# aleflabo/MoCoDAD

Hardware: AMD Instinct MI355X
Metric: pose-clips/sec (whole node) @ noise_steps=10, 5 seeds; AUC vs ref (higher is better)
Workload: dtype f32

## Files before the change

### mocodad_amd/csrc/mcd_device.hpp

```cpp

#pragma once
#include <hip/hip_runtime.h>
#include <stdint.h>
#include <string.h>
#include <stdlib.h>
#include <math.h>
#include <string>
#include <vector>
#include <unordered_map>
#include <utility>
#include <type_traits>
#include <atomic>

#include "../../include/mocodad_hip.h"
#include "mcd_chain.hpp"

namespace mcd {

typedef float f32x4 __attribute__((ext_vector_type(4)));
typedef float f32x2 __attribute__((ext_vector_type(2)));
typedef const float __attribute__((address_space(4))) cfloat;
typedef const float __attribute__((address_space(1))) gfloat;
typedef const f32x4 __attribute__((address_space(1))) gf32x4;
__device__ __forceinline__ gfloat* as_global(const float* p) { return (gfloat*)p; }
// ... 218 lines not shown
    static constexpr int UNITS = NB * CB * NQ;
    static constexpr int PER = (UNITS + NWAVES - 1) / NWAVES;
    static constexpr int NR = (KS * T + 15) / 16;
    static constexpr bool SAMEQ = NQ == 3 && UNITS == 12 && NWAVES == 8;
    static_assert(T > 12 || PER == 1 || UNITS % NWAVES == 0 || SAMEQ, "mix units: a partial round of units (see MixCfg::QX)");
    __host__ __device__ static constexpr int unit_of(int wave, int round) {
        if constexpr (SAMEQ) {
            if (wave < 4) return (wave >> 1) + NQ * ((wave & 1) * 2 + round);
            return round == 0 ? 2 + NQ * (wave - 4) : -1;
        } else {
            const int u = wave + round * NWAVES;
            return u < UNITS ? u : -1;
        }
    }
};
template <int CIN, int V, int T, int NB>
struct MixCoef {
    using M = MixCfg<CIN, V, T, NB>;
    float tq[M::QC][M::NR], aop[M::QC][M::MT][M::KS];
    __device__ __forceinline__ void load(const float* tqd, const float* af, int wave, int lane) {
        load_unit(tqd, af, M::unit_of(wave, 0), lane);
    }
    __device__ __forceinline__ void load_at(const float* tqd, const float* af, int lane) {
        static_assert(M::QC == 1, "one output frame per unit");
        gfloat* tqd_g = as_global(tqd);
        gfloat* af_g = as_global(af);
#pragma unroll
        for (int r = 0; r < M::NR; ++r) tq[0][r] = tqd_g[r * 64 + lane];
#pragma unroll
        for (int mt = 0; mt < M::MT; ++mt)
// ... 321 lines not shown

template <int MT, int NT>
struct Tiling {
    static constexpr int MW = MT > NWAVES ? MT / NWAVES : 1;
    static constexpr int NG = MT > NWAVES ? 1 : NWAVES / MT;
    static constexpr int MAXN = (NT + NG - 1) / NG;
};
template <int MT, int KQ>
__device__ __forceinline__ void load_afrags(const float4* __restrict__ wp, int wave, int lane, float4 (&a)[KQ], int mi = 0) {
    const float* wpl = reinterpret_cast<const float*>(wp + (((wave + mi * NWAVES) % MT) * KQ) * 64 + lane);
#pragma unroll
    for (int kq = 0; kq < KQ; ++kq) a[kq] = load_global4(wpl + kq * 256);
}

struct NoPre { static constexpr bool none = true; };
template <int MT, int NT, int KQ1, int KQ2, bool IDRES, bool FORCE = false, bool DUAL = FORCE, bool SLOTK = false, class Epi, class Pre = NoPre>
__device__ __forceinline__ void gemm_tiles(const float4 (&a)[KQ1 + KQ2], const float* __restrict__ b1, int cs1,
                                           const float* __restrict__ b2, int cs2, int wave, int lane, Epi&& epi, int mi = 0,
                                           const float4 cinit = make_float4(0.f, 0.f, 0.f, 0.f), Pre&& pre = Pre{}) {
    constexpr bool HASPRE = !std::is_same_v<std::decay_t<Pre>, NoPre>;
    constexpr int NG = Tiling<MT, NT>::NG;
    constexpr int MAXN = Tiling<MT, NT>::MAXN;
    const int mt = (wave + mi * NWAVES) % MT, ng = MT > NWAVES ? 0 : wave / MT;
    if (NWAVES % MT != 0 && MT <= NWAVES && ng >= NG) return;
    const int j = lane & 15, g = lane >> 4;
    const int c0 = mt * 16 + 4 * g;
    const int col0 = ng * 16 + j;
    const float* const p1b = b1 + __mul24(col0, cs1) + 4 * g;
    const float* const p2b = b2 + __mul24(col0, cs2) + 4 * g;
    constexpr int KQ = KQ1 + KQ2;
    constexpr int DEPTH0 = KQ < 3 ? KQ : 3;
    auto one_tile = [&](auto ii) {
        constexpr int i = decltype(ii)::value;
        const int col = col0 + i * NG * 16;
        f32x4 c = {cinit.x, cinit.y, cinit.z, cinit.w};
        const float* p1 = p1b + i * NG * 16 * cs1;
        const float* p2 = p2b + i * NG * 16 * cs2;
        if (IDRES) {
            const float4 r = *reinterpret_cast<const float4*>(p2 - 4 * g + c0);
            c[0] = r.x; c[1] = r.y; c[2] = r.z; c[3] = r.w;
        }
        auto rd = [&](auto kk) {
            constexpr int kq = decltype(kk)::value;
            return *reinterpret_cast<const float4*>(kq < KQ1 ? p1 + kq * 16 : p2 + (kq - KQ1) * 16);
// ... 161 lines not shown
}

struct NoHook { __device__ __forceinline__ void operator()() const {} };

template <int KQ>
struct LayerAfr {
    float4 a[KQ];
    float4 bcur;
    template <int MT, bool U32 = false>
    __device__ __forceinline__ void load(const float* wb, const LayerW& lw, int wave, int lane) {
        load_afrags<MT, KQ>(reinterpret_cast<const float4*>(wptr<U32>(wb, lw.wp)), wave, lane, a);
        bcur = load_global4(wptr<U32>(wb, lw.bias) + (wave % MT) * 16 + 4 * (lane >> 4));
    }
};

template <int CIN, int COUT, int V, bool RES, bool HASEMB, int T, int NB, bool FORCE = false, int CSX = cs_of(CIN), bool SLOTSEL = false, class H1, class H2>
__device__ __forceinline__ void layer_generic(const float* wb, const LayerW lw, const MixCoef<CIN, V, T, NB>& mc,
                                              const float* __restrict__ in, float* __restrict__ z, float* __restrict__ out,
                                              const float* __restrict__ embl, int wave, int lane, Prof& prof, int prof_id,
                                              H1&& pre_gemm, H2&& pre_barrier,
                                              const LayerAfr<(CIN / 16) * (RES ? 2 : 1)>* pre_afr = nullptr, const StageRow* rows = nullptr) {
    constexpr int MT = ceil16(COUT) / 16;
    constexpr int COLS = NB * T * V;
    constexpr int NT = ceil16(COLS) / 16;
    constexpr int TV = T * V;
    constexpr int CSI = cs_of(CIN), CSO = cs_of(COUT);
    constexpr int KQ1 = CIN / 16, KQ2 = RES ? CIN / 16 : 0;
    float4 afr[KQ1 + KQ2];
    const int trs = 8 + 8 * ((prof_id - 32) / 3);
    prof.trace(trs + 0);
    constexpr bool TSEL = SLOTSEL && HASEMB && NB == 2 && T == 3;
    constexpr bool ROWS = TSEL && MixCfg<CIN, V, T, NB>::QC == 1;
    const float* bias = wptr<TSEL>(wb, lw.bias);
    float4 bcur;
    if (pre_afr != nullptr) {
#pragma unroll
        for (int k = 0; k < KQ1 + KQ2; ++k) afr[k] = pre_afr->a[k];
        bcur = pre_afr->bcur;
    } else {
        load_afrags<MT, KQ1 + KQ2>(reinterpret_cast<const float4*>(wptr<TSEL>(wb, lw.wp)), wave, lane, afr);
        bcur = load_global4(bias + (wave % MT) * 16 + 4 * (lane >> 4));
    }
    mix_stage<CIN, V, T, NB, FORCE, HASEMB, ROWS>(in, CSX, mc, wptr<TSEL>(wb, lw.tq), wptr<TSEL>(wb, lw.am), wave, lane,
                             ZeroInit{},
                             [&](int n, int q, int w, auto c, auto v) {
                                 if constexpr (ROWS) {
                                     const unsigned za = c.ob + 4u * (unsigned)(__mul24(w, CSI) + c.j);
                                     if constexpr (std::is_same_v<decltype(v), f32x4>) lds_store4(za, v[0], v[1], v[2], v[3]);
                                     else *(lds_float*)(uintptr_t)za = v;
                                 } else {
                                 float* zp = (z + (n * (T * V) * CSI + q * (V * CSI) + c.cb16)) + (__mul24(w, CSI) + c.j);
                                 if constexpr (std::is_same_v<decltype(v), f32x4>) lds_store4(lds_addr(zp), v[0], v[1], v[2], v[3]);
                                 else *zp = v;
                                 }
                             }, rows);
    prof.trace(trs + 1);
    pre_gemm();
    bsync();
// ... 56 lines not shown
    auto epi = [&](auto ti, int col, int c0, f32x4 acc, int, int ng, auto... pe) {
        if (COUT % 16 == 0 || c0 < COUT) {
            float4 e = make_float4(0.f, 0.f, 0.f, 0.f);
            if constexpr (sizeof...(pe) > 0) e = (pe, ...);
            else if constexpr (HASEMB) e = emb_of(ti, col, ng);
            f32x2 t0 = f32x2{acc[0], acc[1]}, t1 = f32x2{acc[2], acc[3]};
            if constexpr (!FOLD) { t0 += f32x2{bcur.x, bcur.y}; t1 += f32x2{bcur.z, bcur.w}; }
            const f32x2 m0 = t0 * slope, m1 = t1 * slope;
            const f32x2 r0 = f32x2{__builtin_amdgcn_fmed3f(t0[0], m0[0], pinf), __builtin_amdgcn_fmed3f(t0[1], m0[1], pinf)} + f32x2{e.x, e.y};
            const f32x2 r1 = f32x2{__builtin_amdgcn_fmed3f(t1[0], m1[0], pinf), __builtin_amdgcn_fmed3f(t1[1], m1[1], pinf)} + f32x2{e.z, e.w};
            constexpr unsigned tile_bytes = 4u * decltype(ti)::value * TILE_STEP * CSO;
            lds_store4(oaddr + tile_bytes, r0[0], r0[1], r1[0], r1[1]);
        }
    };
    prof.trace(trs + 3);
    if constexpr (EPRE) gemm_tiles<MT, NT, KQ1, KQ2, !RES, FORCE, FORCE, TSEL>(afr, z, CSI, in, CSX, wave, lane, epi, 0, FOLD ? bcur : make_float4(0.f, 0.f, 0.f, 0.f), emb_of);
    else gemm_tiles<MT, NT, KQ1, KQ2, !RES, FORCE, FORCE, TSEL>(afr, z, CSI, in, CSX, wave, lane, epi, 0, FOLD ? bcur : make_float4(0.f, 0.f, 0.f, 0.f));
#pragma unroll
    for (int mi = 1; mi < Tiling<MT, NT>::MW; ++mi) {
        load_afrags<MT, KQ1 + KQ2>(reinterpret_cast<const float4*>(wptr<TSEL>(wb, lw.wp)), wave, lane, afr, mi);
        bcur = load_global4(bias + ((wave + mi * NWAVES) % MT) * 16 + 4 * (lane >> 4));
        set_bases(mi);
        if constexpr (EHOIST) e_pre = lds_load4(eaddr);
        if constexpr (EPRE) gemm_tiles<MT, NT, KQ1, KQ2, !RES, FORCE, FORCE, TSEL>(afr, z, CSI, in, CSX, wave, lane, epi, mi, FOLD ? bcur : make_float4(0.f, 0.f, 0.f, 0.f), emb_of);
        else gemm_tiles<MT, NT, KQ1, KQ2, !RES, FORCE, FORCE, TSEL>(afr, z, CSI, in, CSX, wave, lane, epi, mi, FOLD ? bcur : make_float4(0.f, 0.f, 0.f, 0.f));
    }
    prof.trace(trs + 4);
    pre_barrier();
#ifdef MCD_PROFILE
    asm volatile("s_waitcnt lgkmcnt(0)" ::: "memory");
#endif
    prof.trace(trs + 5);
    bsync();
    prof.trace(trs + 6);
    prof.mark(prof_id + 1);
}
template <int CIN, int COUT, int V, bool RES, bool HASEMB, int T, int NB>
__device__ __forceinline__ void layer_generic(const float* wb, const LayerW lw, const float* __restrict__ in,
                                              float* __restrict__ z, float* __restrict__ out,
                                              const float* __restrict__ embl, int wave, int lane, Prof& prof, int prof_id) {
    MixCoef<CIN, V, T, NB> mc;
    mc.load(wb + lw.tq, wb + lw.am, wave, lane);
    layer_generic<CIN, COUT, V, RES, HASEMB, T, NB>(wb, lw, mc, in, z, out, embl, wave, lane, prof, prof_id, NoHook{}, NoHook{});
}

template <int L, int T, int NB>
using LMix = MixCoef<layer_desc(L).cin, layer_desc(L).V, T, NB>;
template <int L>
using LAfr = LayerAfr<(layer_desc(L).cin / 16) * (layer_desc(L).res ? 2 : 1)>;
template <int L, bool U32 = false>
__device__ __forceinline__ void load_lafr(LAfr<L>& A, const float* wb, int wave, int lane) {
    A.template load<ceil16(layer_desc(L).cout) / 16, U32>(wb, layer_w(wb, L), wave, lane);
}
template <int L, int T, int NB, bool FORCE = false, int CSX = cs_of(layer_desc(L).cin), class H1, class H2>
__device__ __forceinline__ void layer_std(const float* wb, const LMix<L, T, NB>& mc, const float* in, float* z, float* out,
                                          const float* emb, int wave, int lane, Prof& prof, H1&& pre_gemm, H2&& pre_barrier,
                                          const LAfr<L>* pre_afr = nullptr, const StageRow* rows = nullptr) {
    constexpr LDesc D = layer_desc(L);
    layer_generic<D.cin, D.cout, D.V, D.res != 0, true, T, NB, FORCE, CSX, true>(wb, layer_w(wb, L), mc, in, z, out, emb + emb_off(L), wave, lane,
                                                               prof, 32 + 3 * L, pre_gemm, pre_barrier, pre_afr, rows);
}

struct EmbRow {
    float4 w[4];
    float b;
    template <bool U32 = false>
    __device__ __forceinline__ void load(const float* wb, int o) {
        const float* we = wptr<U32>(wb, tab_i(wb, TAB_WE));
#pragma unroll
        for (int q = 0; q < 4; ++q) w[q] = load_global4(we + o * EDIM + 4 * q);
        b = as_global(wptr<U32>(wb, tab_i(wb, TAB_BE)))[o];
    }
};
template <int NB>
// ... 82 lines not shown
```

### mocodad_amd/csrc/mcd_score_kernel.hpp

```cpp
#pragma once
#include "mcd_device.hpp"
#include "mcd_encode_kernel.hpp"
#include "mcd_stage_table.hpp"

namespace mcd {

template <int T, int NB, int MINW, bool LT = false>
__global__ __launch_bounds__(NTHREADS, MINW) void score_kernel(const ScoreParams P) {
    using PL = Plan<T, NB>;
    constexpr int TV17 = T * 17;
    constexpr int COLS17 = NB * TV17;
    extern __shared__ __attribute__((aligned(16))) float smem[];
    float* const RG = smem;
    float* const XT = smem + PL::O_XT;
    float* const EMB = smem + PL::O_EMB;
    float* const E10 = smem + PL::O_E10;
    float* const SEN = E10 + 32;
    float* const ZN = smem + PL::O_ZN;
    int* const WM = reinterpret_cast<int*>(smem + PL::O_WM);
    float* const BIA = smem + PL::O_BIA;
    int* const UPD = reinterpret_cast<int*>(smem + PL::O_UPD);
    float* const ZO = smem + PL::O_ZO;

    const int tid0 = threadIdx.x;
    int tid = tid0;
    int lane = tid & 63;
    int wave = __builtin_amdgcn_readfirstlane(tid >> 6);
    Prof prof;
    prof.off();
#ifdef MCD_PROFILE
    const unsigned long long wg_t0 = __builtin_amdgcn_s_memrealtime();
#endif
    if (P.phase > 0 && blockIdx.x * 2 >= gridDim.x) {
        const unsigned long long t0 = __builtin_readcyclecounter();
        while (__builtin_readcyclecounter() - t0 < (unsigned long long)P.phase * 1024ull) __builtin_amdgcn_s_sleep(32);
    }
    if (P.phase < -15) {
// ... 3 lines not shown
    }
    const int grp = blockIdx.x / P.split, part = blockIdx.x - grp * P.split;
    const int win0 = grp * NB;
    const int Tx = P.n_corrupt;
    auto window_of = [&](int n) { const int b = win0 + n; return b < P.B ? b : P.B - 1; };
    if (threadIdx.x < NB) {
        const int b = window_of(threadIdx.x);
        WM[threadIdx.x] = P.win_mask ? P.win_mask[b] : (int)P.fixed_mask;
        WM[4 + threadIdx.x] = b;
        if (threadIdx.x == 0) { WM[8] = 0; WM[9] = -1; }
    }
    if (threadIdx.x >= 128 && threadIdx.x < 128 + NB * T) {
        const int i = threadIdx.x - 128, n = i / T, t = i % T;
        const int fixed = P.win_mask ? P.win_mask[window_of(n)] : (int)P.fixed_mask;
        const int k = P.win_mask ? (((fixed >> t) & 1) ? -1 : 0) : P.upd_of[t];
        UPD[i] = k < 0 ? -1 : (n * T + (P.win_mask ? t : P.pos_of[k])) * 17;
    }
    static_assert(NB <= 4 && T <= 16 && NB * T <= 16, "tail index packing: 4 bits (chain, frame) | 2 bits chain | 4 bits frame");
    int* const TT = reinterpret_cast<int*>(ZO + PL::ZO);
    float* const CE = reinterpret_cast<float*>(TT + PL::TT);
    float* const LOSSB = CE + PL::CE;
    float* const EXW = LOSSB + PL::LOSS;
    if constexpr (MINW >= 4) {
        if (threadIdx.x == 0) {
            int sh = P.prio_shift;
            if (sh > 0 && P.tune) {
                const int sig = (int)gridDim.x * 1009 + P.S * 31 + P.ns;
                const int ticks = P.tune[1];
                if (P.tune[0] == sig && ticks > 0) {
                    const unsigned v = (unsigned)(((unsigned long long)(unsigned)ticks * (unsigned)(P.prio_rounds > 0 ? P.prio_rounds : 1)) / 6u) | 1u;
                    sh = 31 - __clz((int)v);
                    if ((v >> (sh > 0 ? sh - 1 : 0)) & 1u) ++sh;
                    sh = sh < 10 ? 10 : (sh > 26 ? 26 : sh);
                }
            }
            UPD[15] = sh;
            UPD[14] = (int)(unsigned)__builtin_amdgcn_s_memrealtime();
        }
    }
    for (int u = threadIdx.x; u < EMB_EXTRA * 17; u += NTHREADS) {
        const int r = u / 17, k = u % 17;
        EXW[r * 20 + k] = k < 16 ? P.wbuf[tab_i(P.wbuf, TAB_WE) + (NTHREADS + r) * EDIM + k] : P.wbuf[tab_i(P.wbuf, TAB_BE) + NTHREADS + r];
    }
    for (int u = threadIdx.x; u < COLS17 * C0; u += NTHREADS) {
        const int col = u / C0, n = col / TV17, t = (col / 17) % T, v = col % 17;
        TT[u] = (n * T + t) | (n << 4) | (t << 6) | (v << 10);
    }
    if (threadIdx.x < 64) BIA[threadIdx.x] = P.wbuf[tab_i(P.wbuf, 6 * F_STRIDE + F_BIAS) + threadIdx.x];
    else if (threadIdx.x < 64 + C0) BIA[threadIdx.x] = P.wbuf[tab_i(P.wbuf, 10 * F_STRIDE + F_BIAS) + threadIdx.x - 64];
    else if (threadIdx.x >= 80 && threadIdx.x < 112) BIA[threadIdx.x] = P.wbuf[tab_i(P.wbuf, 8 * F_STRIDE + F_BIAS) + threadIdx.x - 80];
    const int CTV = C0 * Tx * 17;
    const int K = P.ns > 2 ? P.ns - 1 : 1;

    if (P.cond_inkernel) {
        static_assert(CondFastLds<T, NB>::FLOATS <= PL::R, "cond_fast_body's region does not fit the work region zeroed for it");
        int enc_solo = -1;
        do {
            for (int u = tid; u < PL::R; u += NTHREADS) smem[u] = 0.f;
            bsync();
            cond_fast_body<T, NB, (NB > 1)>(P.wbuf, P.dv, [&](int t) { return P.cond_idx[t]; }, P.seg_len, smem, win0, P.B, CE, nullptr, enc_solo);
// ... 97 lines not shown
            float xv[C0];
#pragma unroll
            for (int c = 0; c < C0; ++c) {
                if (solo >= 0 && n != solo) {
                    xv[c] = 0.f;
                } else if (mode == 1) {
                    xv[c] = x_in ? x_in[((b * C0 + c) * T + t) * 17 + v] : 0.f;
                } else if ((fixed >> t) & 1) {
                    xv[c] = load_coord(dv, b, c, fm_src(P, t), v, seg_len);
                } else {
                    const int e = (c * Tx + fm_tx(P, fixed, t)) * 17 + v;
                    if (noise) xv[c] = noise[((size_t)(s * K + 0) * Bq + b) * CTV + e];
                    else xv[c] = philox_normal(seed, (unsigned)e, 0u, (unsigned)s, (unsigned)(first_window + b));
                }
            }
            XT[u * 4 + 0] = xv[0];
            XT[u * 4 + 1] = xv[1];
        }
    }
    bsync();
    {
        EmbRow er;
        er.load(P.wbuf, tid_s);
        silu_row(i_first, tid_s);
        bsync();
        emb_compute<NB>(er, EXW, SEN, EMB, E10 + (i_first & 1) * 16, tid_s);
        bsync();
    }
    LMix<0, T, NB> mc0;
    mc0.load(P.wbuf + tab_i(P.wbuf, F_TQ), P.wbuf + tab_i(P.wbuf, F_AM), wave, lane);
    constexpr bool WEARLY = T <= 4;
    LAfr<0> A0;
    if constexpr (WEARLY) load_lafr<0>(A0, P.wbuf, wave, lane);
    stage_rows_of(wave);
    srows(r0, srow::L0);
    for (int sidx = i_first; sidx >= i_last; --sidx) {
        const float* srow = P.step_table + sidx * (4 + EDIM);
        const float* wb = P.wbuf;
        asm volatile("" : "+s"(wb));
        tid = tid0;
        asm volatile("" : "+v"(tid));
        lane = tid & 63;
        wave = __builtin_amdgcn_readfirstlane(tid >> 6);
        stage_rows_of(wave);
        if constexpr (MINW >= 4) {
// ... 17 lines not shown
                float z[4] = {0.f, 0.f, 0.f, 0.f};
                const int fixed = WM[n];
                const int solo = NB > 1 ? WM[9] : -1;
                if (!((fixed >> t) & 1) && (solo < 0 || n == solo)) {
                    const int b = WM[4 + n];
                    const int tx = fm_tx(P, fixed, t);
                    const int k = P.ns - sidx;
                    if (P.noise) {
                        const float* zp = P.noise + ((size_t)(s * K + k) * P.B + b) * CTV + tx * 17 + v0;
                        z[0] = zp[0]; z[1] = zp[Tx * 17];
                        if (v0 + 1 < 17) { z[2] = zp[1]; z[3] = zp[Tx * 17 + 1]; }
                    } else {
                        philox_normal4(P.seed, (unsigned)(tx * 9 + (v0 >> 1)), (unsigned)k, (unsigned)s, (unsigned)(P.first_window + b), z);
                    }
                }
                float* zo = ZN + ((n * T + t) * 17 + v0) * C0;
                zo[0] = z[0]; zo[1] = z[1];
                if (v0 + 1 < 17) { zo[2] = z[2]; zo[3] = z[3]; }
            }
        };
        noise_part(tid);
        STAGE(0);
        STAGE(1);
#ifdef MCD_PROFILE
        prof.bidx = 0;
        prof.tr_on = prof.won && prof.tr && s == part && sidx == i_first - 1;
        prof.trace(0);
#endif
        auto mixload = [&](auto& mc, int l) { mc.load(wptr<TSEL>(wb, tab_i(wb, l * F_STRIDE + F_TQ)), wptr<TSEL>(wb, tab_i(wb, l * F_STRIDE + F_AM)), wave, lane); };
        auto rsload = [&](auto& rc, int r) { rc.load(wptr<TSEL>(wb, tab_i(wb, TAB_RSW + r)), wptr<TSEL>(wb, tab_i(wb, TAB_RSB + r)), lane); };
        auto wptrb = [&](unsigned bytes) { return reinterpret_cast<const float*>(reinterpret_cast<const char*>(wb) + bytes); };
        auto mixrow_at = [&](auto& mc, int tq, int am, const StageRow& r) { mc.load_at(wptrb(4u * (unsigned)tq + r.tq_o), wptrb(4u * (unsigned)am + r.af_o), lane); };
        auto mixrows = [&](auto& mc, int l, auto& r, int id) {
            if constexpr (TSEL) { srows(r, id); mixrow_at(mc, tab_i(wb, l * F_STRIDE + F_TQ), tab_i(wb, l * F_STRIDE + F_AM), r[0]); }
            else mixload(mc, l);
        };
        auto mix_early = mixload;
        auto rs_early = rsload;
        NoHook nohook;
        constexpr bool EARLY2 = LOWO || T == 6;
        LMix<1, T, NB> mc1;
        LAfr<1> A1; LAfr<2> A2; LAfr<3> A3; LAfr<4> A4; LAfr<5> A5; LAfr<7> A7; LAfr<9> A9;
        auto wearly = [&](auto& A, auto lc) { if constexpr (WEARLY) load_lafr<decltype(lc)::value, TSEL>(A, wb, wave, lane); };
#define MCD_LC(l) std::integral_constant<int, l>{}
        layer_std<0, T, NB, LOWO, 4>(wb, mc0, XT, RG + PL::L0_z, RG + PL::L0_out, EMB, wave, lane, prof,
                            [&] { mixrows(mc1, 1, r1, srow::L1); }, [&] { wearly(A1, MCD_LC(1)); }, WEARLY ? &A0 : nullptr, r0);
        STAGE(2);
        lt_dump(0, RG + PL::L0_out, 20, 16, 17);
        lt_inject(1, RG + PL::L1_in, 20, 16, 17);
        LMix<2, T, NB> mc2;
        silu_row(sidx > 0 ? sidx - 1 : 0, tid - NZ_T0);
        layer_std<1, T, NB, LOWO>(wb, mc1, RG + PL::L1_in, RG + PL::L1_z, RG + PL::L1_out, EMB, wave, lane, prof,
                            [&] { mixrows(mc2, 2, r2, srow::L2); }, [&] { wearly(A2, MCD_LC(2)); }, WEARLY ? &A1 : nullptr, r1);
        STAGE(3);
        lt_dump(1, RG + PL::L1_out, 36, 32, 17);
        lt_inject(2, RG + PL::L2_in, 36, 32, 17);
        RsCoef<32, 17, 12, T, NB, true> rc1;
        LMix<3, T, NB> mc3;
        constexpr bool SQ12 = !LT && MixCfg<32, 12, T, NB>::SAMEQ;
        layer_std<2, T, NB, LOWO>(wb, mc2, RG + PL::L2_in, RG + PL::L2_z, RG + PL::L2_out, EMB, wave, lane, prof,
// ... 175 lines not shown
            if constexpr (!SQ12) bsync();
            prof.mark(32 + 3 * 8);
            STAGE(14);
            lt_dump(8, RG + PL::L8_p + 32, 68, 32, 12);
            lt_inject(14, RG + PL::L8_p + 32, 68, 32, 12);
            if constexpr (!EARLY2) mixrows(mc9, 9, r9, srow::L9);
            resample_stage<32, 12, 17, T, NB, false, true, LOWO, SQ12, TSEL && SQ12>(RG + PL::L8_p + 32, 68, RG + PL::UP2_out, 36, rc4, skip1, wave, lane, rup2);
        }
        wearly(A9, MCD_LC(9));
        bsync();
        STAGE(15);
        lt_dump(14, RG + PL::UP2_out, 36, 32, 17);
        lt_inject(9, RG + PL::L9_in, 36, 32, 17);
        {
            const LayerW lw = layer_w(wb, 10);
            MixCoef<16, 17, T, NB> mc10;
            EmbRow ef;
            auto ef_load = [&] { ef.template load<TSEL>(wb, tid); };
            layer_std<9, T, NB, LOWO>(wb, mc9, RG + PL::L9_in, RG + PL::L9_z, RG + PL::L9_out, EMB, wave, lane, prof,
                                [&] {
                                    srows(r10, srow::L10);
                                    if constexpr (TSEL) mixrow_at(mc10, lw.tq, lw.am, r10[0]);
                                    else mc10.load(wptr<TSEL>(wb, lw.tq), wptr<TSEL>(wb, lw.am), wave, lane);
                                    ef_load();
                                }, nohook, WEARLY ? &A9 : nullptr, r9);
            STAGE(16);
            lt_dump(9, RG + PL::L9_out, 36, 32, 17);
            lt_inject(10, RG + PL::L10_in, 36, 32, 17);
            const float ca = srow[0], cb = srow[1], csg = srow[2];
            float* Pb = RG + PL::L10_p;
            {
                const int r = wave & 3;
                const cfloat* w4 = (const cfloat*)(wptr<TSEL>(wb, lw.wp) + r * 32);
                for (int cblk = wave >> 2; cblk * 64 < COLS17; cblk += NWAVES / 4) {
                    const int col = cblk * 64 + lane;
                    if (col < COLS17) {
                        const float* xp = RG + PL::L10_in + col * 36;
                        f32x2 acc2 = {0.f, 0.f};
#pragma unroll
                        for (int q = 0; q < 8; ++q) {
                            const float4 x = *reinterpret_cast<const float4*>(xp + 4 * q);
                            acc2 = f32x2{w4[4 * q + 0], w4[4 * q + 1]} * f32x2{x.x, x.y} + acc2;
                            acc2 = f32x2{w4[4 * q + 2], w4[4 * q + 3]} * f32x2{x.z, x.w} + acc2;
                        }
                        Pb[col * 20 + r] = acc2[0] + acc2[1];
                    }
                }
            }
            STAGE(18);
            emb_compute<NB>(ef, EXW, SEN, EMB, E10 + ((sidx - 1) & 1) * 16, tid);
            STAGE(19);
            bsync();
            STAGE(20);
            const float slope10 = lw.slope;
            const bool single = P.mode == 1, zadd = sidx > 1;
            const int e10_off = (sidx & 1) * 16;
            mix_stage<16, 17, T, NB, LOWO, true, TSEL>(Pb, 20, mc10, wptr<TSEL>(wb, lw.tq), wptr<TSEL>(wb, lw.am), wave, lane,
                                     ZeroInit{},
                                     [&](int n, int t, int w, auto c, auto val) {
                                         if constexpr (TSEL) {
                                             lds_float* zo = (lds_float*)(uintptr_t)c.ob;
                                             if constexpr (std::is_same_v<decltype(val), f32x4>) {
                                                 if (c.j == 0) *(lds_f32x2*)(zo + w * C0) = f32x2{val[0], val[1]};
                                             } else {
                                                 if (c.j < C0) zo[w * C0 + c.j] = val;
                                             }
                                         } else
                                         if constexpr (std::is_same_v<decltype(val), f32x4>) {
                                             if (c.j == 0) *reinterpret_cast<float2*>(ZO + ((n * T + t) * 17 + w) * C0) = make_float2(val[0], val[1]);
                                         } else {
                                             if (c.j < C0) ZO[((n * T + t) * 17 + w) * C0 + c.j] = val;
                                         }
                                     }, r10);
            bsync();
            constexpr int TAIL_IT = (COLS17 * C0 + NTHREADS - 1) / NTHREADS;
            float xn_t[TAIL_IT];
            int dst_t[TAIL_IT];
#pragma unroll
            for (int it = 0; it < TAIL_IT; ++it) {
                const int u = tid + it * NTHREADS;
                dst_t[it] = -1;
                xn_t[it] = 0.f;
                if (u < COLS17 * C0) {
                    const int c = u % C0, col = u / C0;
                    const int tt = TT[u];
                    const int n = (tt >> 4) & 3, t = (tt >> 6) & 15, v = tt >> 10;
                    const float x = XT[col * 4 + c];
                    const float l10 = prelu(ZO[u] + Pb[col * 20 + C0 + c] + BIA[64 + c], slope10) + E10[e10_off + n * 4 + c];
                    const float eps = l10 + x;
                    if constexpr (LT) {
                        const int b = win0 + n;
                        if (P.lt_stage == 10 && b < P.B) P.lt_out[(((size_t)b * C0 + c) * T + t) * 17 + v] = l10;
                    }
                    if (single) {
                        const int b = win0 + n;
                        if (b < P.B && P.eps_out) P.eps_out[(((size_t)b * C0 + c) * T + t) * 17 + v] = eps;
                    } else {
                        const int cbase = UPD[tt & 15];
                        if (cbase >= 0) {
                            const int colp = cbase + v;
                            const float z = zadd ? ZN[colp * C0 + c] : 0.f;
                            xn_t[it] = ca * (XT[colp * 4 + c] - cb * eps) + csg * z;
                            dst_t[it] = colp * 4 + c;
                        }
                    }
                }
            }
            if (P.upd_shift) bsync();
#pragma unroll
            for (int it = 0; it < TAIL_IT; ++it)
                if (dst_t[it] >= 0) XT[dst_t[it]] = xn_t[it];
            srows(r0, srow::L0);
            if constexpr (TSEL) mixrow_at(mc0, tab_i(wb, F_TQ), tab_i(wb, F_AM), r0[0]);
            else mc0.load(wptr<TSEL>(wb, tab_i(wb, F_TQ)), wptr<TSEL>(wb, tab_i(wb, F_AM)), wave, lane);
            wearly(A0, MCD_LC(0));
// ... 17 lines not shown
        float* loss_out = Q->loss_out;
        const bool wmask = Q->win_mask != nullptr;
        for (int u = tid_s; u < NB * per; u += NTHREADS) {
            const int n = u / per, e = u % per;
            const int c = e / (Tx * 17), tx = (e / 17) % Tx, v = e % 17;
            const int solo = NB > 1 ? WM[9] : -1;
            const bool valid = win0 + n < Bq && (solo < 0 || n == solo);
            const int b = WM[4 + n];
            int tu = P.pos_of[tx];
            if (wmask) {
                const int fixed = WM[n];
                int cnt = 0;
                for (int t = 0; t < T; ++t)
                    if (!((fixed >> t) & 1)) { if (cnt == tx) tu = t; ++cnt; }
            }
            const float x0 = XT[((n * T + tu) * 17 + v) * 4 + c];
            const float gt = load_coord(dv, b, c, fm_src(P, tu), v, seg_len);
            const float d = fabsf(x0 - gt);
            float l;
            if (loss_fn == MCD_LOSS_SMOOTH_L1) l = d < 1.f ? 0.5f * d * d : d - 0.5f;
            else if (loss_fn == MCD_LOSS_L1) l = d;
            else l = d * d;
            RED[u] = l;
            if (valid && pose_out) pose_out[(size_t)(b * Sq + s) * per + e] = x0;
        }
        bsync();
        float* PART = RED + NB * per;
        if (tid_s < NB * 8) {
            const int n = tid_s >> 3, p8 = tid_s & 7;
            float sum = 0.f;
            for (int e = p8; e < per; e += 8) sum += RED[n * per + e];
// ... 66 lines not shown
```

### mocodad_amd/csrc/mcd_stage_table.hpp

```cpp
#pragma once
#include "mcd_device.hpp"

namespace mcd {

namespace srow { enum { L0 = 0, L1 = 1, L2 = 2, DN1 = 4, L3 = 6, L8 = 8, UP2 = 10, L9 = 12, L10 = 14, NROWS = 16 }; }

template <int T, int NB>
struct StageTabGen {
    static_assert(T == 3 && NB == 2 && NWAVES == 8, "the stage table is generated for the 3-frame x 2-chain kernel of 8 waves");
    using PL = Plan<T, NB>;
    using M16 = MixCfg<16, 17, T, NB>;
    using M17 = MixCfg<32, 17, T, NB>;
    using M12 = MixCfg<32, 12, T, NB>;
    static_assert(M16::QC == 1 && M16::UNITS == 6 && M16::PER == 1 && M17::SAMEQ && M12::SAMEQ && M17::PER == 2 && M12::PER == 2, "unit maps the rows are generated for");
    enum { L0 = srow::L0, L1 = srow::L1, L2 = srow::L2, DN1 = srow::DN1, L3 = srow::L3, L8 = srow::L8, UP2 = srow::UP2, L9 = srow::L9, L10 = srow::L10, NROWS = srow::NROWS };
    struct Tab { StageRow r[NWAVES][NROWS]; };

    struct Unit { int n, cb, q; };
    template <class M>
    static constexpr Unit unit(int wave, int round) {
        const int um = M::unit_of(wave, round);
        const int u = um < 0 ? 0 : um;
        const int rest = u / M::NQ;
        return Unit{rest / M::CB, rest % M::CB, (u % M::NQ) * M::QC};
    }
    template <class M>
    static constexpr StageRow mix_row(int wave, int round, int V, int in, int cs_in, int out, int cs_out, int aux = 0, int aux2 = 0) {
        const Unit u = unit<M>(wave, round);
        return StageRow{4u * (unsigned)(in + u.n * (T * V) * cs_in + u.cb * 16),
                        4u * (unsigned)(out + u.n * (T * V) * cs_out + u.q * (V * cs_out) + u.cb * 16),
                        4u * (unsigned)(aux + u.n * EMB_STRIDE + u.cb * 16), 4u * (unsigned)(aux2 + u.cb * 16),
                        4u * (unsigned)(u.q * M::NR * 64), 4u * (unsigned)(u.q * M::MT * M::KS * 64), 0u, 0u};
    }
    static constexpr StageRow rs_row(int wave, int slot, int in, int vin, int cs_in, int out, int vout, int cs_out) {
        const Unit u = unit<M12>(wave, slot);
        const int nt = u.n * T + u.q;
        return StageRow{4u * (unsigned)(in + nt * vin * cs_in + u.cb * 16), 4u * (unsigned)(out + nt * vout * cs_out + u.cb * 16), 0u, 0u, 0u, 0u, 0u, 0u};
    }
    static constexpr Tab make() {
        Tab t{};
        for (int w = 0; w < NWAVES; ++w) {
            StageRow* r = t.r[w];
            r[L0] = mix_row<M16>(w, 0, 17, PL::O_XT, 4, PL::L0_z, 20);
            r[L1] = mix_row<M16>(w, 0, 17, PL::L1_in, 20, PL::L1_z, 20);
            r[L10] = mix_row<M16>(w, 0, 17, PL::L10_p, 20, PL::O_ZO, 2);
            for (int k = 0; k < 2; ++k) {
                r[L2 + k] = mix_row<M17>(w, k, 17, PL::L2_in, 36, PL::L2_z, 36);
                r[L9 + k] = mix_row<M17>(w, k, 17, PL::L9_in, 36, PL::L9_z, 36);
                r[L3 + k] = mix_row<M12>(w, k, 12, PL::L3_in, 36, PL::L3_z, 36);
                r[L8 + k] = mix_row<M12>(w, k, 12, PL::L8_p, 68, PL::L8_p + 32, 68, PL::O_EMB + emb_off(8), PL::O_BIA + 80);
                r[DN1 + k] = rs_row(w, k, PL::L2_out, 17, 36, PL::DN1_out, 12, 36);
                r[UP2 + k] = rs_row(w, k, PL::L8_p + 32, 12, 68, PL::UP2_out, 17, 36);
            }
        }
        return t;
    }
};
template <int T, int NB>
struct StageTab : StageTabGen<T, NB> {
    using G = StageTabGen<T, NB>;
// ... 18 lines not shown
        for (int n = 0; n < NB; ++n)
            for (int cb = 0; cb < ncb; ++cb)
                for (int q = 0; q < T; ++q) {
                    int hits = 0;
                    for (int w = 0; w < NWAVES; ++w)
                        for (int k = 0; k < rounds; ++k) {
                            if (rounds == 1 ? w >= 6 : (k == 1 && w >= 4)) continue;
                            const StageRow& r = tab.r[w][row + k];
                            if (r.in_b == in0 + n * in_n + q * in_q + cb * 64u && r.out_b == out0 + n * out_n + q * out_q + cb * 64u &&
                                (tq_q == 0u || (r.tq_o == q * tq_q && r.af_o == q * af_q))) ++hits;
                        }
                    if (hits != 1) return false;
                }
        return true;
    }
    static constexpr bool in_plan() {
        for (int w = 0; w < NWAVES; ++w)
            for (int i = 0; i < G::NROWS; ++i) {
                const StageRow& r = tab.r[w][i];
                if (r.in_b % 16 || r.out_b % 8 || r.aux_b % 16 || r.aux2_b % 16) return false;
                if (r.in_b >= PL::BYTES || r.out_b >= PL::BYTES || r.aux_b >= PL::BYTES || r.aux2_b >= PL::BYTES) return false;
            }
        return true;
    }
};
template <int T, int NB>
constexpr bool stage_tab_checked() {
    using S = StageTab<T, NB>;
    using PL = Plan<T, NB>;
    constexpr unsigned TV17 = T * 17, TV12 = T * 12;
    static_assert(S::sameq_closed_form(), "SAMEQ unit map: not the closed form the rows were checked against");
    static_assert(S::in_plan(), "a stage-table row points outside the LDS plan or is misaligned");
    static_assert(S::covers(S::L0, 1, 1, 4u * PL::O_XT, 4u * TV17 * 4, 0u, 4u * PL::L0_z, 4u * TV17 * 20, 4u * 17 * 20, 256u, 4u * 2 * 5 * 64), "layer 0 rows");
    static_assert(S::covers(S::L1, 1, 1, 4u * PL::L1_in, 4u * TV17 * 20, 0u, 4u * PL::L1_z, 4u * TV17 * 20, 4u * 17 * 20, 256u, 4u * 2 * 5 * 64), "layer 1 rows");
    static_assert(S::covers(S::L10, 1, 1, 4u * PL::L10_p, 4u * TV17 * 20, 0u, 4u * PL::O_ZO, 4u * TV17 * 2, 4u * 17 * 2, 256u, 4u * 2 * 5 * 64), "layer 10 rows");
    static_assert(S::covers(S::L2, 2, 2, 4u * PL::L2_in, 4u * TV17 * 36, 0u, 4u * PL::L2_z, 4u * TV17 * 36, 4u * 17 * 36, 256u, 4u * 2 * 5 * 64), "layer 2 rows");
    static_assert(S::covers(S::L9, 2, 2, 4u * PL::L9_in, 4u * TV17 * 36, 0u, 4u * PL::L9_z, 4u * TV17 * 36, 4u * 17 * 36, 256u, 4u * 2 * 5 * 64), "layer 9 rows");
    static_assert(S::covers(S::L3, 2, 2, 4u * PL::L3_in, 4u * TV12 * 36, 0u, 4u * PL::L3_z, 4u * TV12 * 36, 4u * 12 * 36, 256u, 4u * 1 * 3 * 64), "layer 3 rows");
    static_assert(S::covers(S::L8, 2, 2, 4u * PL::L8_p, 4u * TV12 * 68, 0u, 4u * (PL::L8_p + 32), 4u * TV12 * 68, 4u * 12 * 68, 256u, 4u * 1 * 3 * 64), "layer 8 rows");
    static_assert(S::covers(S::DN1, 2, 2, 4u * PL::L2_out, 4u * TV17 * 36, 4u * 17 * 36, 4u * PL::DN1_out, 4u * TV12 * 36, 4u * 12 * 36), "down1 rows");
    static_assert(S::covers(S::UP2, 2, 2, 4u * (PL::L8_p + 32), 4u * TV12 * 68, 4u * 12 * 68, 4u * PL::UP2_out, 4u * TV17 * 36, 4u * 17 * 36), "up2 rows");
    return true;
}

}
```

Measured before the change: 505,500.

## Pack both chains' coordinates into one channel block for input and output layers

Interleaves the two chains' 2-channel pose coordinates in one 4*NB-wide channel group, so the layer-0 and layer-10 mix stages run as a single-chain (NB=1) mix with 3 units instead of 6. The XT/ZN/ZO indexing, stage table rows and GEMM B-operand addressing all change to the packed layout. The aim is to halve the mix work on the sparse 2-channel layers. It adds index arithmetic, a wave swap for load balance, and layout complexity across several stages.

```diff
diff --git a/mocodad_amd/csrc/mcd_device.hpp b/mocodad_amd/csrc/mcd_device.hpp
--- a/mocodad_amd/csrc/mcd_device.hpp
+++ b/mocodad_amd/csrc/mcd_device.hpp
@@ -256,6 +256,10 @@
         }
     }
 };
+#ifndef MCD_PK_SWAP
+#define MCD_PK_SWAP 1
+#endif
+__host__ __device__ constexpr int pk_wave(int wave) { return MCD_PK_SWAP ? (wave == 2 ? 3 : wave == 3 ? 2 : wave) : wave; }
 template <int CIN, int V, int T, int NB>
 struct MixCoef {
     using M = MixCfg<CIN, V, T, NB>;
@@ -607,7 +611,7 @@
 }
 
 struct NoPre { static constexpr bool none = true; };
-template <int MT, int NT, int KQ1, int KQ2, bool IDRES, bool FORCE = false, bool DUAL = FORCE, bool SLOTK = false, class Epi, class Pre = NoPre>
+template <int MT, int NT, int KQ1, int KQ2, bool IDRES, bool FORCE = false, bool DUAL = FORCE, bool SLOTK = false, int PKR = 0, class Epi, class Pre = NoPre>
 __device__ __forceinline__ void gemm_tiles(const float4 (&a)[KQ1 + KQ2], const float* __restrict__ b1, int cs1,
                                            const float* __restrict__ b2, int cs2, int wave, int lane, Epi&& epi, int mi = 0,
                                            const float4 cinit = make_float4(0.f, 0.f, 0.f, 0.f), Pre&& pre = Pre{}) {
@@ -619,8 +623,12 @@
     const int j = lane & 15, g = lane >> 4;
     const int c0 = mt * 16 + 4 * g;
     const int col0 = ng * 16 + j;
-    const float* const p1b = b1 + __mul24(col0, cs1) + 4 * g;
-    const float* const p2b = b2 + __mul24(col0, cs2) + 4 * g;
+    static_assert(PKR == 0 || (MAXN == 1 && !DUAL && !IDRES && KQ1 == 1 && KQ2 == 1 && NT * 16 <= 2 * PKR + 16),
+                  "packed chains: one tile per wave (a tile's rows are not a fixed step apart), two chains, one k-group per operand");
+    const int pn = PKR > 0 && col0 >= PKR ? 1 : 0;
+    const int prow = PKR > 0 ? min(col0 - pn * PKR, PKR - 1) : col0;
+    const float* const p1b = b1 + __mul24(prow, cs1) + 4 * (g + pn);
+    const float* const p2b = b2 + __mul24(prow, cs2) + 4 * (g + pn);
     constexpr int KQ = KQ1 + KQ2;
     constexpr int DEPTH0 = KQ < 3 ? KQ : 3;
     auto one_tile = [&](auto ii) {
@@ -812,8 +820,8 @@
     }
 };
 
-template <int CIN, int COUT, int V, bool RES, bool HASEMB, int T, int NB, bool FORCE = false, int CSX = cs_of(CIN), bool SLOTSEL = false, class H1, class H2>
-__device__ __forceinline__ void layer_generic(const float* wb, const LayerW lw, const MixCoef<CIN, V, T, NB>& mc,
+template <int CIN, int COUT, int V, bool RES, bool HASEMB, int T, int NB, bool FORCE = false, int CSX = cs_of(CIN), bool SLOTSEL = false, bool PK = false, class H1, class H2>
+__device__ __forceinline__ void layer_generic(const float* wb, const LayerW lw, const MixCoef<CIN, V, T, PK ? 1 : NB>& mc,
                                               const float* __restrict__ in, float* __restrict__ z, float* __restrict__ out,
                                               const float* __restrict__ embl, int wave, int lane, Prof& prof, int prof_id,
                                               H1&& pre_gemm, H2&& pre_barrier,
@@ -828,7 +836,9 @@
     const int trs = 8 + 8 * ((prof_id - 32) / 3);
     prof.trace(trs + 0);
     constexpr bool TSEL = SLOTSEL && HASEMB && NB == 2 && T == 3;
-    constexpr bool ROWS = TSEL && MixCfg<CIN, V, T, NB>::QC == 1;
+    constexpr int NBM = PK ? 1 : NB;
+    static_assert(!PK || (CIN == 16 && RES && NB * 4 <= 16 && CSX == 4 * NB), "packed chains: 4 channels (x0, x1, 0, 0) per chain in one 16-channel block");
+    constexpr bool ROWS = TSEL && MixCfg<CIN, V, T, NBM>::QC == 1;
     const float* bias = wptr<TSEL>(wb, lw.bias);
     float4 bcur;
     if (pre_afr != nullptr) {
@@ -839,7 +849,7 @@
         load_afrags<MT, KQ1 + KQ2>(reinterpret_cast<const float4*>(wptr<TSEL>(wb, lw.wp)), wave, lane, afr);
         bcur = load_global4(bias + (wave % MT) * 16 + 4 * (lane >> 4));
     }
-    mix_stage<CIN, V, T, NB, FORCE, HASEMB, ROWS>(in, CSX, mc, wptr<TSEL>(wb, lw.tq), wptr<TSEL>(wb, lw.am), wave, lane,
+    mix_stage<CIN, V, T, NBM, FORCE, HASEMB, ROWS>(in, CSX, mc, wptr<TSEL>(wb, lw.tq), wptr<TSEL>(wb, lw.am), PK ? pk_wave(wave) : wave, lane,
                              ZeroInit{},
                              [&](int n, int q, int w, auto c, auto v) {
                                  if constexpr (ROWS) {
@@ -926,16 +936,16 @@
         }
     };
     prof.trace(trs + 3);
-    if constexpr (EPRE) gemm_tiles<MT, NT, KQ1, KQ2, !RES, FORCE, FORCE, TSEL>(afr, z, CSI, in, CSX, wave, lane, epi, 0, FOLD ? bcur : make_float4(0.f, 0.f, 0.f, 0.f), emb_of);
-    else gemm_tiles<MT, NT, KQ1, KQ2, !RES, FORCE, FORCE, TSEL>(afr, z, CSI, in, CSX, wave, lane, epi, 0, FOLD ? bcur : make_float4(0.f, 0.f, 0.f, 0.f));
+    if constexpr (EPRE) gemm_tiles<MT, NT, KQ1, KQ2, !RES, FORCE, FORCE, TSEL, PK ? TV : 0>(afr, z, CSI, in, CSX, wave, lane, epi, 0, FOLD ? bcur : make_float4(0.f, 0.f, 0.f, 0.f), emb_of);
+    else gemm_tiles<MT, NT, KQ1, KQ2, !RES, FORCE, FORCE, TSEL, PK ? TV : 0>(afr, z, CSI, in, CSX, wave, lane, epi, 0, FOLD ? bcur : make_float4(0.f, 0.f, 0.f, 0.f));
 #pragma unroll
     for (int mi = 1; mi < Tiling<MT, NT>::MW; ++mi) {
         load_afrags<MT, KQ1 + KQ2>(reinterpret_cast<const float4*>(wptr<TSEL>(wb, lw.wp)), wave, lane, afr, mi);
         bcur = load_global4(bias + ((wave + mi * NWAVES) % MT) * 16 + 4 * (lane >> 4));
         set_bases(mi);
         if constexpr (EHOIST) e_pre = lds_load4(eaddr);
-        if constexpr (EPRE) gemm_tiles<MT, NT, KQ1, KQ2, !RES, FORCE, FORCE, TSEL>(afr, z, CSI, in, CSX, wave, lane, epi, mi, FOLD ? bcur : make_float4(0.f, 0.f, 0.f, 0.f), emb_of);
-        else gemm_tiles<MT, NT, KQ1, KQ2, !RES, FORCE, FORCE, TSEL>(afr, z, CSI, in, CSX, wave, lane, epi, mi, FOLD ? bcur : make_float4(0.f, 0.f, 0.f, 0.f));
+        if constexpr (EPRE) gemm_tiles<MT, NT, KQ1, KQ2, !RES, FORCE, FORCE, TSEL, PK ? TV : 0>(afr, z, CSI, in, CSX, wave, lane, epi, mi, FOLD ? bcur : make_float4(0.f, 0.f, 0.f, 0.f), emb_of);
+        else gemm_tiles<MT, NT, KQ1, KQ2, !RES, FORCE, FORCE, TSEL, PK ? TV : 0>(afr, z, CSI, in, CSX, wave, lane, epi, mi, FOLD ? bcur : make_float4(0.f, 0.f, 0.f, 0.f));
     }
     prof.trace(trs + 4);
     pre_barrier();
@@ -964,12 +974,12 @@
 __device__ __forceinline__ void load_lafr(LAfr<L>& A, const float* wb, int wave, int lane) {
     A.template load<ceil16(layer_desc(L).cout) / 16, U32>(wb, layer_w(wb, L), wave, lane);
 }
-template <int L, int T, int NB, bool FORCE = false, int CSX = cs_of(layer_desc(L).cin), class H1, class H2>
-__device__ __forceinline__ void layer_std(const float* wb, const LMix<L, T, NB>& mc, const float* in, float* z, float* out,
+template <int L, int T, int NB, bool FORCE = false, int CSX = cs_of(layer_desc(L).cin), bool PK = false, class H1, class H2>
+__device__ __forceinline__ void layer_std(const float* wb, const LMix<L, T, PK ? 1 : NB>& mc, const float* in, float* z, float* out,
                                           const float* emb, int wave, int lane, Prof& prof, H1&& pre_gemm, H2&& pre_barrier,
                                           const LAfr<L>* pre_afr = nullptr, const StageRow* rows = nullptr) {
     constexpr LDesc D = layer_desc(L);
-    layer_generic<D.cin, D.cout, D.V, D.res != 0, true, T, NB, FORCE, CSX, true>(wb, layer_w(wb, L), mc, in, z, out, emb + emb_off(L), wave, lane,
+    layer_generic<D.cin, D.cout, D.V, D.res != 0, true, T, NB, FORCE, CSX, true, PK>(wb, layer_w(wb, L), mc, in, z, out, emb + emb_off(L), wave, lane,
                                                                prof, 32 + 3 * L, pre_gemm, pre_barrier, pre_afr, rows);
 }
 
diff --git a/mocodad_amd/csrc/mcd_score_kernel.hpp b/mocodad_amd/csrc/mcd_score_kernel.hpp
--- a/mocodad_amd/csrc/mcd_score_kernel.hpp
+++ b/mocodad_amd/csrc/mcd_score_kernel.hpp
@@ -21,6 +21,11 @@
     float* const BIA = smem + PL::O_BIA;
     int* const UPD = reinterpret_cast<int*>(smem + PL::O_UPD);
     float* const ZO = smem + PL::O_ZO;
+    constexpr bool PK = T == 3 && NB == 2;
+    static_assert(!PK || NB * 2 <= 16, "packed chains: two coordinates per chain in one 16-channel block");
+    constexpr int NBM = PK ? 1 : NB;
+    auto xcol = [](int n, int t, int v) { return PK ? (t * 17 + v) * NB + n : (n * T + t) * 17 + v; };
+    constexpr int XVS = PK ? NB : 1;
 
     const int tid0 = threadIdx.x;
     int tid = tid0;
@@ -54,7 +59,7 @@
         const int i = threadIdx.x - 128, n = i / T, t = i % T;
         const int fixed = P.win_mask ? P.win_mask[window_of(n)] : (int)P.fixed_mask;
         const int k = P.win_mask ? (((fixed >> t) & 1) ? -1 : 0) : P.upd_of[t];
-        UPD[i] = k < 0 ? -1 : (n * T + (P.win_mask ? t : P.pos_of[k])) * 17;
+        UPD[i] = k < 0 ? -1 : xcol(n, P.win_mask ? t : P.pos_of[k], 0);
     }
     static_assert(NB <= 4 && T <= 16 && NB * T <= 16, "tail index packing: 4 bits (chain, frame) | 2 bits chain | 4 bits frame");
     int* const TT = reinterpret_cast<int*>(ZO + PL::ZO);
@@ -83,7 +88,8 @@
         EXW[r * 20 + k] = k < 16 ? P.wbuf[tab_i(P.wbuf, TAB_WE) + (NTHREADS + r) * EDIM + k] : P.wbuf[tab_i(P.wbuf, TAB_BE) + NTHREADS + r];
     }
     for (int u = threadIdx.x; u < COLS17 * C0; u += NTHREADS) {
-        const int col = u / C0, n = col / TV17, t = (col / 17) % T, v = col % 17;
+        const int col = u / C0;
+        const int n = PK ? col % NB : col / TV17, t = PK ? col / (NB * 17) : (col / 17) % T, v = PK ? (col / NB) % 17 : col % 17;
         TT[u] = (n * T + t) | (n << 4) | (t << 6) | (v << 10);
     }
     if (threadIdx.x < 64) BIA[threadIdx.x] = P.wbuf[tab_i(P.wbuf, 6 * F_STRIDE + F_BIAS) + threadIdx.x];
@@ -211,8 +217,8 @@
                     else xv[c] = philox_normal(seed, (unsigned)e, 0u, (unsigned)s, (unsigned)(first_window + b));
                 }
             }
-            XT[u * 4 + 0] = xv[0];
-            XT[u * 4 + 1] = xv[1];
+            XT[xcol(n, t, v) * 4 + 0] = xv[0];
+            XT[xcol(n, t, v) * 4 + 1] = xv[1];
         }
     }
     bsync();
@@ -224,8 +230,8 @@
         emb_compute<NB>(er, EXW, SEN, EMB, E10 + (i_first & 1) * 16, tid_s);
         bsync();
     }
-    LMix<0, T, NB> mc0;
-    mc0.load(P.wbuf + tab_i(P.wbuf, F_TQ), P.wbuf + tab_i(P.wbuf, F_AM), wave, lane);
+    LMix<0, T, NBM> mc0;
+    mc0.load(P.wbuf + tab_i(P.wbuf, F_TQ), P.wbuf + tab_i(P.wbuf, F_AM), PK ? pk_wave(wave) : wave, lane);
     constexpr bool WEARLY = T <= 4;
     LAfr<0> A0;
     if constexpr (WEARLY) load_lafr<0>(A0, P.wbuf, wave, lane);
@@ -273,9 +279,9 @@
                         philox_normal4(P.seed, (unsigned)(tx * 9 + (v0 >> 1)), (unsigned)k, (unsigned)s, (unsigned)(P.first_window + b), z);
                     }
                 }
-                float* zo = ZN + ((n * T + t) * 17 + v0) * C0;
+                float* zo = ZN + xcol(n, t, v0) * C0;
                 zo[0] = z[0]; zo[1] = z[1];
-                if (v0 + 1 < 17) { zo[2] = z[2]; zo[3] = z[3]; }
+                if (v0 + 1 < 17) { zo[XVS * C0] = z[2]; zo[XVS * C0 + 1] = z[3]; }
             }
         };
         noise_part(tid);
@@ -302,7 +308,7 @@
         LAfr<1> A1; LAfr<2> A2; LAfr<3> A3; LAfr<4> A4; LAfr<5> A5; LAfr<7> A7; LAfr<9> A9;
         auto wearly = [&](auto& A, auto lc) { if constexpr (WEARLY) load_lafr<decltype(lc)::value, TSEL>(A, wb, wave, lane); };
 #define MCD_LC(l) std::integral_constant<int, l>{}
-        layer_std<0, T, NB, LOWO, 4>(wb, mc0, XT, RG + PL::L0_z, RG + PL::L0_out, EMB, wave, lane, prof,
+        layer_std<0, T, NB, LOWO, 4 * XVS, PK>(wb, mc0, XT, RG + PL::L0_z, RG + PL::L0_out, EMB, wave, lane, prof,
                             [&] { mixrows(mc1, 1, r1, srow::L1); }, [&] { wearly(A1, MCD_LC(1)); }, WEARLY ? &A0 : nullptr, r0);
         STAGE(2);
         lt_dump(0, RG + PL::L0_out, 20, 16, 17);
@@ -508,7 +514,7 @@
         lt_inject(9, RG + PL::L9_in, 36, 32, 17);
         {
             const LayerW lw = layer_w(wb, 10);
-            MixCoef<16, 17, T, NB> mc10;
+            MixCoef<16, 17, T, NBM> mc10;
             EmbRow ef;
             auto ef_load = [&] { ef.template load<TSEL>(wb, tid); };
             layer_std<9, T, NB, LOWO>(wb, mc9, RG + PL::L9_in, RG + PL::L9_z, RG + PL::L9_out, EMB, wave, lane, prof,
@@ -537,7 +543,8 @@
                             acc2 = f32x2{w4[4 * q + 0], w4[4 * q + 1]} * f32x2{x.x, x.y} + acc2;
                             acc2 = f32x2{w4[4 * q + 2], w4[4 * q + 3]} * f32x2{x.z, x.w} + acc2;
                         }
-                        Pb[col * 20 + r] = acc2[0] + acc2[1];
+                        if constexpr (PK) Pb[(col >= TV17 ? (col - TV17) * 20 + 4 : col * 20) + r] = acc2[0] + acc2[1];
+                        else Pb[col * 20 + r] = acc2[0] + acc2[1];
                     }
                 }
             }
@@ -549,15 +556,16 @@
             const float slope10 = lw.slope;
             const bool single = P.mode == 1, zadd = sidx > 1;
             const int e10_off = (sidx & 1) * 16;
-            mix_stage<16, 17, T, NB, LOWO, true, TSEL>(Pb, 20, mc10, wptr<TSEL>(wb, lw.tq), wptr<TSEL>(wb, lw.am), wave, lane,
+            mix_stage<16, 17, T, NBM, LOWO, true, TSEL>(Pb, 20, mc10, wptr<TSEL>(wb, lw.tq), wptr<TSEL>(wb, lw.am), wave, lane,
                                      ZeroInit{},
                                      [&](int n, int t, int w, auto c, auto val) {
-                                         if constexpr (TSEL) {
+                                         if constexpr (PK) {
+                                             static_assert(TSEL, "the packed mix takes its rows from the stage table");
                                              lds_float* zo = (lds_float*)(uintptr_t)c.ob;
                                              if constexpr (std::is_same_v<decltype(val), f32x4>) {
-                                                 if (c.j == 0) *(lds_f32x2*)(zo + w * C0) = f32x2{val[0], val[1]};
+                                                 if (c.j < 4 * NB) *(lds_f32x2*)(zo + (w * (NB * C0) + (c.j >> 1))) = f32x2{val[0], val[1]};
                                              } else {
-                                                 if (c.j < C0) zo[w * C0 + c.j] = val;
+                                                 if (c.j < 4 * NB && (c.j & 3) < C0) zo[w * (NB * C0) + (c.j >> 2) * C0 + (c.j & 3)] = val;
                                              }
                                          } else
                                          if constexpr (std::is_same_v<decltype(val), f32x4>) {
@@ -580,7 +588,7 @@
                     const int tt = TT[u];
                     const int n = (tt >> 4) & 3, t = (tt >> 6) & 15, v = tt >> 10;
                     const float x = XT[col * 4 + c];
-                    const float l10 = prelu(ZO[u] + Pb[col * 20 + C0 + c] + BIA[64 + c], slope10) + E10[e10_off + n * 4 + c];
+                    const float l10 = prelu(ZO[u] + Pb[(PK ? (col / NB) * 20 + 4 * (col % NB) : col * 20) + C0 + c] + BIA[64 + c], slope10) + E10[e10_off + n * 4 + c];
                     const float eps = l10 + x;
                     if constexpr (LT) {
                         const int b = win0 + n;
@@ -592,7 +600,7 @@
                     } else {
                         const int cbase = UPD[tt & 15];
                         if (cbase >= 0) {
-                            const int colp = cbase + v;
+                            const int colp = cbase + v * XVS;
                             const float z = zadd ? ZN[colp * C0 + c] : 0.f;
                             xn_t[it] = ca * (XT[colp * 4 + c] - cb * eps) + csg * z;
                             dst_t[it] = colp * 4 + c;
@@ -640,7 +648,7 @@
                 for (int t = 0; t < T; ++t)
                     if (!((fixed >> t) & 1)) { if (cnt == tx) tu = t; ++cnt; }
             }
-            const float x0 = XT[((n * T + tu) * 17 + v) * 4 + c];
+            const float x0 = XT[xcol(n, tu, v) * 4 + c];
             const float gt = load_coord(dv, b, c, fm_src(P, tu), v, seg_len);
             const float d = fabsf(x0 - gt);
             float l;
diff --git a/mocodad_amd/csrc/mcd_stage_table.hpp b/mocodad_amd/csrc/mcd_stage_table.hpp
--- a/mocodad_amd/csrc/mcd_stage_table.hpp
+++ b/mocodad_amd/csrc/mcd_stage_table.hpp
@@ -10,9 +10,10 @@
     static_assert(T == 3 && NB == 2 && NWAVES == 8, "the stage table is generated for the 3-frame x 2-chain kernel of 8 waves");
     using PL = Plan<T, NB>;
     using M16 = MixCfg<16, 17, T, NB>;
+    using M16P = MixCfg<16, 17, T, 1>;
     using M17 = MixCfg<32, 17, T, NB>;
     using M12 = MixCfg<32, 12, T, NB>;
-    static_assert(M16::QC == 1 && M16::UNITS == 6 && M16::PER == 1 && M17::SAMEQ && M12::SAMEQ && M17::PER == 2 && M12::PER == 2, "unit maps the rows are generated for");
+    static_assert(M16::QC == 1 && M16::UNITS == 6 && M16::PER == 1 && M16P::QC == 1 && M16P::UNITS == 3 && M17::SAMEQ && M12::SAMEQ && M17::PER == 2 && M12::PER == 2, "unit maps the rows are generated for");
     enum { L0 = srow::L0, L1 = srow::L1, L2 = srow::L2, DN1 = srow::DN1, L3 = srow::L3, L8 = srow::L8, UP2 = srow::UP2, L9 = srow::L9, L10 = srow::L10, NROWS = srow::NROWS };
     struct Tab { StageRow r[NWAVES][NROWS]; };
 
@@ -41,9 +42,9 @@
         Tab t{};
         for (int w = 0; w < NWAVES; ++w) {
             StageRow* r = t.r[w];
-            r[L0] = mix_row<M16>(w, 0, 17, PL::O_XT, 4, PL::L0_z, 20);
+            r[L0] = mix_row<M16P>(pk_wave(w), 0, 17, PL::O_XT, 4 * NB, PL::L0_z, 20);
             r[L1] = mix_row<M16>(w, 0, 17, PL::L1_in, 20, PL::L1_z, 20);
-            r[L10] = mix_row<M16>(w, 0, 17, PL::L10_p, 20, PL::O_ZO, 2);
+            r[L10] = mix_row<M16P>(w, 0, 17, PL::L10_p, 20, PL::O_ZO, 2 * NB);
             for (int k = 0; k < 2; ++k) {
                 r[L2 + k] = mix_row<M17>(w, k, 17, PL::L2_in, 36, PL::L2_z, 36);
                 r[L9 + k] = mix_row<M17>(w, k, 17, PL::L9_in, 36, PL::L9_z, 36);
@@ -92,6 +93,17 @@
                 }
         return true;
     }
+    static constexpr bool covers_packed(int row, bool swapped, unsigned in0, unsigned out0, unsigned out_q, unsigned tq_q, unsigned af_q) {
+        for (int q = 0; q < T; ++q) {
+            int hits = 0;
+            for (int wu = 0; wu < T; ++wu) {
+                const StageRow& r = tab.r[swapped ? pk_wave(wu) : wu][row];
+                if (r.in_b == in0 && r.out_b == out0 + q * out_q && r.tq_o == q * tq_q && r.af_o == q * af_q) ++hits;
+            }
+            if (hits != 1) return false;
+        }
+        return true;
+    }
     static constexpr bool in_plan() {
         for (int w = 0; w < NWAVES; ++w)
             for (int i = 0; i < G::NROWS; ++i) {
@@ -109,9 +121,9 @@
     constexpr unsigned TV17 = T * 17, TV12 = T * 12;
     static_assert(S::sameq_closed_form(), "SAMEQ unit map: not the closed form the rows were checked against");
     static_assert(S::in_plan(), "a stage-table row points outside the LDS plan or is misaligned");
-    static_assert(S::covers(S::L0, 1, 1, 4u * PL::O_XT, 4u * TV17 * 4, 0u, 4u * PL::L0_z, 4u * TV17 * 20, 4u * 17 * 20, 256u, 4u * 2 * 5 * 64), "layer 0 rows");
+    static_assert(S::covers_packed(S::L0, true, 4u * PL::O_XT, 4u * PL::L0_z, 4u * 17 * 20, 256u, 4u * 2 * 5 * 64), "layer 0 rows");
     static_assert(S::covers(S::L1, 1, 1, 4u * PL::L1_in, 4u * TV17 * 20, 0u, 4u * PL::L1_z, 4u * TV17 * 20, 4u * 17 * 20, 256u, 4u * 2 * 5 * 64), "layer 1 rows");
-    static_assert(S::covers(S::L10, 1, 1, 4u * PL::L10_p, 4u * TV17 * 20, 0u, 4u * PL::O_ZO, 4u * TV17 * 2, 4u * 17 * 2, 256u, 4u * 2 * 5 * 64), "layer 10 rows");
+    static_assert(S::covers_packed(S::L10, false, 4u * PL::L10_p, 4u * PL::O_ZO, 4u * 17 * 2 * NB, 256u, 4u * 2 * 5 * 64), "layer 10 rows");
     static_assert(S::covers(S::L2, 2, 2, 4u * PL::L2_in, 4u * TV17 * 36, 0u, 4u * PL::L2_z, 4u * TV17 * 36, 4u * 17 * 36, 256u, 4u * 2 * 5 * 64), "layer 2 rows");
     static_assert(S::covers(S::L9, 2, 2, 4u * PL::L9_in, 4u * TV17 * 36, 0u, 4u * PL::L9_z, 4u * TV17 * 36, 4u * 17 * 36, 256u, 4u * 2 * 5 * 64), "layer 9 rows");
     static_assert(S::covers(S::L3, 2, 2, 4u * PL::L3_in, 4u * TV12 * 36, 0u, 4u * PL::L3_z, 4u * TV12 * 36, 4u * 12 * 36, 256u, 4u * 1 * 3 * 64), "layer 3 rows");
```

After: 506,900, median of 5. No clear change (+0.3%).
